# Mingtzge/PVE-MCC_for_unsignalized_intersection

Measured on AMD Instinct MI355X. Metric: env-steps/sec (vehicles x envs x steps/s) at 128 veh x 4096 envs, higher is better.
Workload: dtype f64

## Files before the change

### pve-mcc_for_unsignalized_intersection_amd/csrc/pve_tick_core.h

```cpp
#pragma once
#include "pve_types.h"
#include <math.h>
#include <string.h>
#include <type_traits>

#if defined(__HIP_DEVICE_COMPILE__)
#define PVE_AS4 __attribute__((address_space(4)))
#else
#define PVE_AS4
#endif
#if defined(__HIPCC__)
#undef PVE_HD
#define PVE_HD __device__ __forceinline__
#define PVE_DEVICE_CODE 1
#else
#define PVE_DEVICE_CODE 0
#endif

namespace pve {

typedef unsigned long long u64;

template <int NW> PVE_HD void vote(u64 *m, int t, bool f)
{
#if PVE_DEVICE_CODE
    u64 b = __ballot(f);
    if ((t & 63) == 0) m[t >> 6] = b;
#else
    if (f) m[t >> 6] |= 1ull << (t & 63);
#endif
}
template <int NW, int N> PVE_HD void vote_many(u64 *const (&m)[N], int t, const bool (&f)[N])
{
#if PVE_DEVICE_CODE
    u64 b[N];
#pragma unroll
    for (int k = 0; k < N; k++) b[k] = __ballot(f[k]);
    if ((t & 63) == 0) {
#pragma unroll
        for (int k = 0; k < N; k++) m[k][t >> 6] = b[k];
    }
#else
    for (int k = 0; k < N; k++) if (f[k]) m[k][t >> 6] |= 1ull << (t & 63);
#endif
}
PVE_HD bool mask_test(const u64 *m, int t) { return (m[t >> 6] >> (t & 63)) & 1ull; }
PVE_HD u64 below_sel(int rel)
{
    return rel >= 64 ? ~0ull : (rel > 0 ? ((1ull << (rel & 63)) - 1ull) : 0ull);
}
PVE_HD int popc_below(u64 w, int rel)
{
    const int r = rel < 0 ? 0 : (rel > 64 ? 64 : rel);
    const int c = __builtin_popcountll(w << ((64 - r) & 63));
    return r == 0 ? 0 : c;
}
template <int NW> PVE_HD int mask_below(const u64 *m, int t)
{
    int c = 0;
#pragma unroll
    for (int k = 0; k < NW; k++) c += popc_below(m[k], t - k * 64);
    return c;
}
template <int NW> PVE_HD int mask_rank(const u64 *m, int t)
{
#if PVE_DEVICE_CODE
    if constexpr (NW <= 2) {
    const u64 w0 = m[0], w1 = m[NW - 1];
    const bool up = NW > 1 && t >= 64;
    const u64 w = up ? w1 : w0;
    int c = (int)__builtin_amdgcn_mbcnt_hi((unsigned)(w >> 32), __builtin_amdgcn_mbcnt_lo((unsigned)w, 0u));
    c += up ? __builtin_popcountll(w0) : 0;
    return c;
    } else {
        static_assert(NW == 4, "mask_rank: 64, 128 or 256 slots");
        const int wi = t >> 6;
        u64 w = m[0];
        int c = 0;
#pragma unroll
        for (int k = 1; k < NW; k++) {
            const u64 mk = m[k];
            c += wi >= k ? __builtin_popcountll(m[k - 1]) : 0;
            w = wi == k ? mk : w;
        }
        return c + (int)__builtin_amdgcn_mbcnt_hi((unsigned)(w >> 32), __builtin_amdgcn_mbcnt_lo((unsigned)w, 0u));
    }
#else
    return mask_below<NW>(m, t);
#endif
}
template <int NW> PVE_HD int mask_count(const u64 *m)
{
    int c = 0;
#pragma unroll
    for (int k = 0; k < NW; k++) c += __builtin_popcountll(m[k]);
    return c;
}
template <int NW> PVE_HD int mask_prev(const u64 *m, int t)
{
    int best = -1;
#pragma unroll
    for (int k = 0; k < NW; k++) {
        const u64 b = m[k] & below_sel(t - k * 64);
        best = b ? (k * 64 + 63 - __builtin_clzll(b | 1ull)) : best;
    }
    return best;
}
PVE_HD void lds_add(int *p, int v)
{
#if PVE_DEVICE_CODE
    atomicAdd(p, v);
#else
    *p += v;
#endif
}
PVE_HD int lds_claim(int *p, int n)
{
#if PVE_DEVICE_CODE
    return atomicAdd(p, n);
#else
    int o = *p; *p += n; return o;
#endif
}
PVE_HD unsigned lds_xchg(unsigned *p, unsigned v)
{
#if PVE_DEVICE_CODE
    return __hip_atomic_exchange(p, v, __ATOMIC_ACQ_REL, __HIP_MEMORY_SCOPE_WORKGROUP);
#else
    const unsigned o = *p; *p = v; return o;
#endif
}
template <class T> PVE_HD void lds_store_relaxed(T *p, T v)
{
#if PVE_DEVICE_CODE
    __hip_atomic_store(p, v, __ATOMIC_RELAXED, __HIP_MEMORY_SCOPE_WORKGROUP);
#else
    *p = v;
#endif
}
template <bool COH, class T> PVE_HD T gld(const T *p)
{
#if PVE_DEVICE_CODE
    if constexpr (COH) {
        static_assert(sizeof(T) == 4 || sizeof(T) == 8, "gld: 4- or 8-byte scalars");
        if constexpr (sizeof(T) == 8) {
            const unsigned long long u = __hip_atomic_load((const unsigned long long *)p, __ATOMIC_RELAXED, __HIP_MEMORY_SCOPE_AGENT);
            T v; __builtin_memcpy(&v, &u, 8); return v;
        } else {
            const unsigned u = __hip_atomic_load((const unsigned *)p, __ATOMIC_RELAXED, __HIP_MEMORY_SCOPE_AGENT);
            T v; __builtin_memcpy(&v, &u, 4); return v;
        }
    } else return *p;
#else
    return *p;
#endif
}
template <class ROW> PVE_HD void gather_state(const ROW *const (&srcs)[NNB + 1], unsigned coh, ROW *dst)
{
#if PVE_DEVICE_CODE
    typedef float v4f __attribute__((ext_vector_type(4)));
    constexpr int CPR = (int)sizeof(ROW) * OBSW / 112;
    constexpr int NC = (NNB + 1) * CPR;
    v4f buf[7];
    auto fetch = [&](int c, v4f (&q)[7]) {
        const ROW *row = srcs[c / CPR];
        const char *sp = (const char *)row + 112 * (c % CPR);
        if (!row) {
#pragma unroll
            for (int i = 0; i < 7; i++) q[i] = v4f{0.f, 0.f, 0.f, 0.f};
        } else if ((coh >> (c / CPR)) & 1u) {
            asm volatile("global_load_dwordx4 %0, %7, off sc1\n\tglobal_load_dwordx4 %1, %7, off offset:16 sc1\n\t"
                         "global_load_dwordx4 %2, %7, off offset:32 sc1\n\tglobal_load_dwordx4 %3, %7, off offset:48 sc1\n\t"
                         "global_load_dwordx4 %4, %7, off offset:64 sc1\n\tglobal_load_dwordx4 %5, %7, off offset:80 sc1\n\t"
                         "global_load_dwordx4 %6, %7, off offset:96 sc1\n\ts_waitcnt vmcnt(0)"
                         : "=&v"(q[0]), "=&v"(q[1]), "=&v"(q[2]), "=&v"(q[3]), "=&v"(q[4]), "=&v"(q[5]), "=&v"(q[6]) : "v"(sp) : "memory");
        } else {
#pragma unroll
            for (int i = 0; i < 7; i++) q[i] = ((const v4f *)sp)[i];
        }
    };
#pragma unroll
    for (int c = 0; c < NC; c++) {
        fetch(c, buf);
        v4f *d4 = (v4f *)((char *)dst + 112 * c);
#pragma unroll
        for (int i = 0; i < 7; i++) d4[i] = buf[i];
    }
#else
    for (int q = 0; q <= NNB; q++)
        for (int k = 0; k < OBSW; k++) dst[q * OBSW + k] = srcs[q] ? srcs[q][k] : (ROW)0;
#endif
}
template <class W> PVE_HD int sidx_at(const W *s, int i)
{
    if constexpr (sizeof(W) == 4) return ((const uint16_t *)s)[2 * i];
    else return s[i];
}
PVE_HD void lds_or(int *p, int v)
{
#if PVE_DEVICE_CODE
    atomicOr(p, v);
#else
    *p |= v;
#endif
}
PVE_HD void lds_and(int *p, int v)
{
#if PVE_DEVICE_CODE
    atomicAnd(p, v);
#else
    *p &= v;
#endif
}
PVE_HD int wave_incl_scan(int t, int x, int *emu_acc)
{
#if PVE_DEVICE_CODE
    x += __builtin_amdgcn_mov_dpp(x, 0x111, 0xf, 0xf, true);
    x += __builtin_amdgcn_mov_dpp(x, 0x112, 0xf, 0xf, true);
    x += __builtin_amdgcn_mov_dpp(x, 0x114, 0xf, 0xf, true);
    x += __builtin_amdgcn_mov_dpp(x, 0x118, 0xf, 0xf, true);
    x += __builtin_amdgcn_update_dpp(0, x, 0x142, 0xa, 0xf, false);
    x += __builtin_amdgcn_update_dpp(0, x, 0x143, 0xc, 0xf, false);
    return x;
#else
    *emu_acc += x;
    return *emu_acc;
#endif
}
#if PVE_DEVICE_CODE
template <int CTRL, int ROW_MASK> PVE_HD double dpp_add_f64(double x)
{
    const int lo = __double2loint(x), hi = __double2hiint(x);
    int slo, shi;
    if (ROW_MASK == 0xf) {
        slo = __builtin_amdgcn_mov_dpp(lo, CTRL, 0xf, 0xf, true);
        shi = __builtin_amdgcn_mov_dpp(hi, CTRL, 0xf, 0xf, true);
    } else {
        slo = __builtin_amdgcn_update_dpp(0, lo, CTRL, ROW_MASK, 0xf, false);
        shi = __builtin_amdgcn_update_dpp(0, hi, CTRL, ROW_MASK, 0xf, false);
    }
    return x + __hiloint2double(shi, slo);
}
#endif
PVE_HD void block_sum(double *red, int t, double x)
{
#if PVE_DEVICE_CODE
    x = dpp_add_f64<0x111, 0xf>(x);
    x = dpp_add_f64<0x112, 0xf>(x);
    x = dpp_add_f64<0x114, 0xf>(x);
    x = dpp_add_f64<0x118, 0xf>(x);
    x = dpp_add_f64<0x142, 0xa>(x);
    x = dpp_add_f64<0x143, 0xc>(x);
    if ((t & 63) == 63) red[t >> 6] = x;
#else
    red[0] += x;
#endif
}

PVE_HD void block_sum_sparse(double *red, int t, bool has, double x)
{
#if PVE_DEVICE_CODE
    if (__builtin_amdgcn_ballot_w64(has) == 0) {
        if ((t & 63) == 63) red[t >> 6] = 0.0;
        return;
    }
#endif
    block_sum(red, t, has ? x : 0.0);
}

#ifdef PVE_SELECT_CLAMPS
PVE_HD double dmax(double a, double b) { return (a > b) ? a : b; }
PVE_HD double dmin(double a, double b) { return (a < b) ? a : b; }
#else
PVE_HD double dmax(double a, double b) { return __builtin_fmax(a, b); }
PVE_HD double dmin(double a, double b) { return __builtin_fmin(a, b); }
#endif

#ifdef PVE_WIDE_INDEX
template <int PER, class T> PVE_HD T *env_at(T *base, int env, int idx) { return base + ((size_t)env * PER + (size_t)idx); }
#else
template <int PER, class T> PVE_HD T *env_at(T *base, int env, int idx)
{
    return (T *)((char *)(base + (size_t)env * PER) + (unsigned)(idx * (int)sizeof(T)));
}
#endif

PVE_HD int mul24(int a, int b)
{
#if PVE_DEVICE_CODE && !defined(PVE_NO_RANGE_ASSUME)
    return __mul24(a, b);
#else
    return a * b;
#endif
}
PVE_HD int mad24(int a, int b, int c)
{
#if PVE_DEVICE_CODE && !defined(PVE_NO_RANGE_ASSUME)
    return __mul24(a, b) + c;
#else
    return a * b + c;
#endif
}

template <int CAP> using slot_t = typename std::conditional<(CAP <= 128), uint8_t, uint16_t>::type;
template <int CAP> constexpr int SLOT_NONE = CAP <= 128 ? 255 : 0xFFFF;
template <int CAP> struct Homes {
    static_assert(CAP <= 128, "HOME: id_info[1] is packed into one byte of h_sv (no HOME build at 256 slots)");
    double h_jerk_sum[CAP], h_closer[CAP];
    int h_id[CAP], h_sv[CAP], h_count[CAP];
};
template <int CAP> struct HomesOff {};
struct HomeRegs { double jerk_sum, closer, vir_dis; int id, sv, count; };
template <int CAP, bool LJ = (CAP == 128), bool HOME_ = false, int POOL_ = (HOME_ ? 304 * CAP / 128 : 5 * CAP)>
struct Shared : std::conditional<HOME_, Homes<CAP>, HomesOff<CAP>>::type {
    static constexpr int NW = CAP / 64;
    static constexpr bool HOME = HOME_;
    static_assert(!HOME_ || (POOL_ * 4 >= 2 * CAP * 4 + CAP + 1 && POOL_ >= CAP && POOL_ % 8 == 0), "HOME: the staging overlays need 2 CAP ints + CAP + 1 bytes of s_idx");
    static constexpr bool PIN_READS = true;
    static constexpr int POOL = POOL_;
    static constexpr bool DIRECT = (CAP == 64);
    static constexpr bool DENSE = true;
    EnvHeader hd;
    double p[CAP], v[CAP + 1], a[CAP + 1];
    union {
        struct { double p1[CAP], v1[CAP]; };
        double u_vd[POOL];
    };
    double virdis[CAP];
    int cnt[CAP];
    alignas(8) unsigned s_idx[DIRECT ? 1 : POOL];
    double s_vd[DIRECT ? POOL : 1];
    alignas(8) uint8_t u_slot[POOL];
    enum { SF_JERK = 0, SF_JERK_SUM, SF_VIR_DIS, SF_CLOSER_P, SF_P, SF_V, SF_A };
    template <int K> PVE_HD double *stf()
    {
        if (HOME) return K == SF_JERK ? u_vd + CAP : (K == SF_P ? p : (K == SF_V ? v : a));
        return K < 4 ? u_vd + (K + 1) * CAP : (K == SF_P ? u_vd : (K == SF_V ? v : a));
    }
    PVE_HD slot_t<CAP> *keep_pre() { return (slot_t<CAP> *)(DIRECT ? (uint8_t *)s_vd + 7 * CAP * 4 : (uint8_t *)s_idx + 2 * CAP * 4); }
    PVE_HD uint8_t *fxcode() { return u_list + CAP; }
    PVE_HD slot_t<CAP> *chain() { return (slot_t<CAP> *)u_slot; }
    template <int K> PVE_HD int *sti()
    {
        if (DIRECT) return (int *)s_vd + K * CAP;
        if (HOME) return K == I_STEP ? (int *)s_idx : (K == I_META ? (int *)s_idx + CAP : cnt);
        return K < 2 ? (int *)s_idx + K * CAP : (K < 4 ? (int *)p + (K - 2) * CAP : (K == 4 ? cnt : (K == 5 ? (int *)u_slot : (int *)(u_list + CAP))));
    }
    int acc_passed_steps, acc_collisions;
    union {
        int16_t pref[NL * 5];
        int16_t hdr[CAP];
    };
    union {
        uint8_t bb[CAP];
        uint8_t rew_ovr[CAP];
    };
    u64 m_alive[NW], m_ctl[NW];
    union {
        int nfin[NL];
        struct {
            u64 m_del[NW], m_fin[NW], m_ctlnow[NW], m_coll[NW];
            union { u64 m_lead[NW]; u64 m_keep[NW]; };
            u64 m_spawn[NW];
        };
    };
    uint8_t s_slot[DIRECT ? POOL : 1];
    union {
        alignas(8) uint8_t u_list[POOL];
        uint8_t lk_slot[POOL];
    };
    union {
        uint8_t mypos[CAP];
        uint8_t cyc_off[CAP];
    };
    uint8_t slot_of[CAP];
    int16_t cstart[NL + 1];
#if !PVE_DEVICE_CODE
    int emu_scan;
#endif
    int16_t loff[NL + 1];
    union {
        alignas(8) int16_t segoff[NL][5];
        struct { double red_reward[NW], red_jerk[NW]; };
    };
    uint8_t lane_of[CAP + 1];
    static constexpr bool HAS_LJ = LJ;
    int lj[HAS_LJ ? CAP + 1 : 1];
    union {
        float xy32[CAP][2];
        double act_next[CAP];
    };
    double tabA[2][4], tabB[2][4], tabC[2][4];
    alignas(4) uint8_t l2lp[NL][4];
    int lead_n;
    static_assert(POOL < (1 << 16), "s_idx: entry | tag << 16");
    static_assert((CAP + 1) * sizeof(slot_t<CAP>) <= POOL, "chain() in u_slot");
    static_assert(HOME_ || 5 * CAP <= POOL, "stf<>(): the EARLY staging doubles in u_vd[0 .. 5 CAP)");
    static_assert(DIRECT || HOME_ || (CAP * 4 <= POOL && CAP + CAP * 4 <= POOL), "sti<5>() in u_slot, sti<6>() in u_list[CAP ..)");
    static_assert(DIRECT ? 7 * CAP * 4 + (CAP + 1) * sizeof(slot_t<CAP>) <= POOL * sizeof(double)
                         : 2 * CAP * 4 + (CAP + 1) * sizeof(slot_t<CAP>) <= POOL * 4, "keep_pre() behind the EARLY staging ints");
};

struct Regs {
    double p, v, a, jerk, jerk_sum, vir_dis, closer_p;
    double a0, a1;
    double reward;
    double kv[NNB];
    int kr[NNB];
    int id, seq, vnum, step, count, meta;
    int lane, j;
    int hdr;
    int hit, coll_seen, coll_fin;
    int alive, ctl, del, fin;
    int cyc;
    int intent, route, ord;
    int mmask;
    int dctl, ds, dlane;
    double dp, djerk, dcloser;
    double act;
    double next_arr;
    double act_nx;
};
struct FinCarry {
    int still, meta;
    int new_slot;
    int ls;
    int sp_slot, sp_id, sp_vnum;
    int sp_int;
    int n_post, n_sp;
    int n_ctl;
};
struct CRegs {
    double p, v, a, jerk, jerk_sum, vir_dis, closer_p;
    int id, seq, vnum, step, count, meta, hdr_word, alive;
    double obsrow[OBSW];
};

PVE_HD void sincos_q1(double x, double &sn, double &cs)
{
    const double hp = 1.5707963267948966;
    const bool fold = x > 0.7853981633974483;
    const double y = fold ? (hp - x) : x;
    const double z = y * y;
    double ps = -7.6471637318198164759e-13;
    ps = ps * z + 1.6059043836821614599e-10;
    ps = ps * z - 2.5052108385441718775e-08;
    ps = ps * z + 2.7557319223985890653e-06;
    ps = ps * z - 1.9841269841269841270e-04;
    ps = ps * z + 8.3333333333333333333e-03;
    ps = ps * z - 1.6666666666666666667e-01;
    const double s1 = y + y * z * ps;
    double pc = 4.7794773323873852974e-14;
    pc = pc * z - 1.1470745597729724714e-11;
    pc = pc * z + 2.0876756987868098979e-09;
    pc = pc * z - 2.7557319223985890653e-07;
    pc = pc * z + 2.4801587301587301587e-05;
    pc = pc * z - 1.3888888888888888889e-03;
    pc = pc * z + 4.1666666666666666667e-02;
    const double c1 = 1.0 - 0.5 * z + z * z * pc;
    sn = fold ? c1 : s1;
    cs = fold ? s1 : c1;
}

#if PVE_DEVICE_CODE
#define PVE_PIN(x) asm volatile("" : "+v"(x))
#else
#define PVE_PIN(x) ((void)0)
#endif

PVE_HD double sel2(double a0, double a1, bool second)
{
#if PVE_DEVICE_CODE
    asm volatile("" : "+s"(a0), "+s"(a1));
#endif
    return second ? a1 : a0;
}
PVE_HD double sel3(const PVE_AS4 double (&a)[3], int i)
{
    double a0 = a[0], a1 = a[1], a2 = a[2];
#if PVE_DEVICE_CODE
    asm volatile("" : "+s"(a0), "+s"(a1), "+s"(a2));
#endif
    return i == 0 ? a0 : (i == 1 ? a1 : a2);
}
PVE_HD double sel4(const PVE_AS4 double (&a)[4], int i)
{
    double a0 = a[0], a1 = a[1], a2 = a[2], a3 = a[3];
#if PVE_DEVICE_CODE
    asm volatile("" : "+s"(a0), "+s"(a1), "+s"(a2), "+s"(a3));
#endif
    return i == 0 ? a0 : (i == 1 ? a1 : (i == 2 ? a2 : a3));
}

PVE_HD void get_xy(const PVE_AS4 Const &c, double p, int lane, double &X, double &Y)
{
    const double cw = c.cw;
    const int m = lane % 3;
    const double Lb = sel2(c.inbox[0], c.inbox[2], m == 2);
    const bool before = p > Lb, inside = !before && p > 0;
    const bool arc = (m != 1) && inside;
    double sn, cs;
    sincos_q1(arc ? ((Lb - p) / Lb * c.arc_k / 2) : 0.0, sn, cs);
    const double p0y = (m == 0) ? cw : 5 * cw, pry = (m == 0) ? -6 * cw : 6 * cw;
    const double p0x = 6 * cw, prx = 6 * cw;
    const double ax = (m == 0) ? (prx + (p0x - prx) * cs - (p0y - pry) * sn) : (prx + (p0x - prx) * cs + (p0y - pry) * sn);
    const double ay = (m == 0) ? (pry + (p0y - pry) * cs + (p0x - prx) * sn) : (pry + (p0y - pry) * cs - (p0x - prx) * sn);
    const double bx = p - Lb + 6 * cw, by = p0y;
    const double ex = (m == 0) ? -cw : 5 * cw;
    const double ey = (m == 0) ? (-6 * cw + p) : (6 * cw - p);
    double x = before ? bx : (inside ? ax : ex);
    double y = before ? by : (inside ? ay : ey);
    if (m == 1) { x = p - 6 * cw; y = 3 * cw; }
    const double rc = sel4(c.rot_cos, lane / 3), rs = sel4(c.rot_sin, lane / 3);
    X = x * rc - y * rs;
    Y = y * rc + x * rs;
}

PVE_HD float frcp(float x)
{
#if PVE_DEVICE_CODE
    return __builtin_amdgcn_rcpf(x);
#else
    return 1.0f / x;
#endif
}
PVE_HD void get_xy_f32(const PVE_AS4 Const &c, double pd, int lane, float &X, float &Y)
{
    const float cw = (float)c.cw, p = (float)pd;
    const int m = lane % 3;
    const float Lb = (float)sel2(c.inbox[0], c.inbox[2], m == 2);
    const bool before = p > Lb, inside = !before && p > 0.f;
    float ra = (m != 1 && inside) ? ((Lb - p) * (1.5707965f * frcp(Lb))) : 0.f;
    const bool fold = ra > 0.78539816f;
    const float y0 = fold ? (1.5707964f - ra) : ra, z = y0 * y0;
    const float s1 = y0 + y0 * z * (-1.6666667e-1f + z * (8.3333338e-3f + z * (-1.9841270e-4f + z * 2.7557319e-6f)));
    const float c1 = 1.f + z * (-0.5f + z * (4.1666668e-2f + z * (-1.3888889e-3f + z * 2.4801587e-5f)));
    const float sn = fold ? c1 : s1, cs = fold ? s1 : c1;
    const float p0y = (m == 0) ? cw : 5.f * cw, pry = (m == 0) ? -6.f * cw : 6.f * cw, prx = 6.f * cw;
    const float ax = (m == 0) ? (prx - (p0y - pry) * sn) : (prx + (p0y - pry) * sn);
    const float ay = pry + (p0y - pry) * cs;
    float x = before ? (p - Lb + 6.f * cw) : (inside ? ax : ((m == 0) ? -cw : 5.f * cw));
    float y = before ? p0y : (inside ? ay : ((m == 0) ? (-6.f * cw + p) : (6.f * cw - p)));
    if (m == 1) { x = p - 6.f * cw; y = 3.f * cw; }
    const int q = lane / 3;
    const bool odd = (q & 1) != 0;
    const float xr = odd ? -y : x, yr = odd ? x : y;
    X = (q & 2) ? -xr : xr;
    Y = (q & 2) ? -yr : yr;
}

PVE_HD double exp_m2_0(double x)
{
    const double k = rint(x * 1.4426950408889634074);
    double r = __builtin_fma(-k, 6.93147180369123816490e-01, x);
    r = __builtin_fma(-k, 1.90821492927058770002e-10, r);
    double p = 1.0 / 479001600.0;
    p = __builtin_fma(p, r, 1.0 / 39916800.0);
    p = __builtin_fma(p, r, 1.0 / 3628800.0);
    p = __builtin_fma(p, r, 1.0 / 362880.0);
    p = __builtin_fma(p, r, 1.0 / 40320.0);
    p = __builtin_fma(p, r, 1.0 / 5040.0);
    p = __builtin_fma(p, r, 1.0 / 720.0);
    p = __builtin_fma(p, r, 1.0 / 120.0);
    p = __builtin_fma(p, r, 1.0 / 24.0);
    p = __builtin_fma(p, r, 1.0 / 6.0);
    p = __builtin_fma(p, r, 0.5);
    p = __builtin_fma(p, r, 1.0);
    p = __builtin_fma(p, r, 1.0);
    return ldexp(p, (int)k);
}
PVE_HD double value_div(double x, double y)
{
#if PVE_DEVICE_CODE
    double r = __builtin_amdgcn_rcp(y);
    r = __builtin_fma(__builtin_fma(-y, r, 1.0), r, r);
    r = __builtin_fma(__builtin_fma(-y, r, 1.0), r, r);
    return x * r;
#else
    return x / y;
#endif
}
PVE_HD double reward_coth_term(double t_distance)
{
    const double u = exp_m2_0(-0.5 * t_distance);
    const double den = u - 1.0;
    return den == 0.0 ? -INFINITY : value_div(u + 1.0, den);
}
PVE_HD double reward_log_term(double z)
{
    int e;
    double m = frexp(z, &e);
    const bool lo = m < 0.70710678118654752;
    m = lo ? m + m : m;
    e = lo ? e - 1 : e;
    const double f = m - 1.0;
    const double s = value_div(f, 2.0 + f);
    const double w = s * s;
    double q = 1.0 / 19.0;
    q = __builtin_fma(q, w, 1.0 / 17.0);
    q = __builtin_fma(q, w, 1.0 / 15.0);
    q = __builtin_fma(q, w, 1.0 / 13.0);
    q = __builtin_fma(q, w, 1.0 / 11.0);
    q = __builtin_fma(q, w, 1.0 / 9.0);
    q = __builtin_fma(q, w, 1.0 / 7.0);
    q = __builtin_fma(q, w, 1.0 / 5.0);
    q = __builtin_fma(q, w, 1.0 / 3.0);
    q = __builtin_fma(q, w, 1.0);
    return __builtin_fma((double)e, 0.69314718055994530942, (s + s) * q);
}

PVE_HD bool key_less(double d1, double v1, int r1, double d2, double v2, int r2)
{
    return d1 < d2 || (d1 == d2 && (v1 < v2 || (v1 == v2 && r1 < r2)));
}

PVE_HD double div_const(double x, double b, double rb)
{
    const double q = x * rb;
    const double r = __builtin_fma(-q, b, x);
    return __builtin_fma(r, rb, q);
}
PVE_HD int brake_needed(const PVE_AS4 Const &c, double p, double v, double fp, double fv)
{
    const double d_safe = v * 0.4 + div_const(v * v - fv * fv, c.two_abs_am, c.inv_two_abs_am) -
                          div_const((v - fv) * c.vm, c.abs_am, c.inv_abs_am);
    return ((fv < v) & (p - fp < d_safe)) ? 1 : 0;
}

PVE_HD int slot_lane(const EnvHeader &hd, int t)
{
    int lane = 0;
#pragma unroll
    for (int L = 1; L < NL; L++) lane += (t >= hd.lane_start[L]) ? 1 : 0;
    return lane;
}

template <int CAP, class ShT = Shared<CAP>> struct Tick {
    typedef ShT Sh;
    static constexpr int NW = CAP / 64;

    template <bool COH = false, bool COHA = false>
    static PVE_HD void ph_load(const PVE_AS4 Const &c, const PVE_AS4 Params &P, int env, int t, Sh &sh, Regs &r,
                               const double *act0 = nullptr, bool use_act0 = false)
    {
        const EnvHeader &gh = P.headers[env];
        {
            const int *src = (const int *)&gh;
            int *dst = (int *)&sh.hd;
            for (int w = t + 2; w < (int)(sizeof(EnvHeader) / 4); w += CAP) dst[w] = gld<COH>(src + w);
        }
        if (t == 0) sh.hd.current_time = gld<COH>(&gh.current_time) + c.deltaT;
        const int N = gld<COH>(&gh.n_alive);
        const size_t g = (size_t)env * CAP + t;
        r.alive = t < N;
        r.jerk = 0;
        r.p = r.v = r.a = r.jerk_sum = r.vir_dis = r.closer_p = 0;
        r.id = r.seq = r.vnum = r.step = r.count = r.meta = 0;
        r.act = 0;
        const double *acts = use_act0 ? act0 : P.actions;
        if (t < 64 || t < N) {
            if (acts) r.act = gld<COHA>(acts + g);
            r.p = gld<COH>(P.f64[F_P] + g); r.v = gld<COH>(P.f64[F_V] + g); r.a = gld<COH>(P.f64[F_A] + g);
            r.meta = gld<COH>(P.i32[I_META] + g); r.step = gld<COH>(P.i32[I_STEP] + g);
            r.jerk_sum = gld<COH>(P.f64[F_JERK_SUM] + g); r.vir_dis = gld<COH>(P.f64[F_VIR_DIS] + g);
            r.closer_p = gld<COH>(P.f64[F_CLOSER_P] + g);
            r.id = gld<COH>(P.i32[I_ID] + g); r.seq = gld<COH>(P.i32[I_SEQ] + g); r.vnum = gld<COH>(P.i32[I_VNUM] + g);
            r.count = gld<COH>(P.i32[I_COUNT] + g);
        }
        sh.cnt[t] = 0;
        if (t == 0) {
            sh.acc_passed_steps = 0; sh.acc_collisions = 0; sh.lead_n = 0;
            sh.v[CAP] = 0; sh.a[CAP] = 0; sh.lane_of[CAP] = 0;
            if constexpr (Sh::HAS_LJ) sh.lj[CAP] = 0;
        }
        if (t < 8) {
            sh.tabA[t >> 2][t & 3] = c.vdA[t >> 2][t & 3];
            sh.tabB[t >> 2][t & 3] = c.vdB[t >> 2][t & 3];
            sh.tabC[t >> 2][t & 3] = c.vdC[t >> 2][t & 3];
        }
        if (t < NL * 4) {
            const int L = c.l2l[t >> 2][t & 3];
            sh.l2lp[t >> 2][t & 3] = (uint8_t)((L < 0 ? 15 : L) | ((c.l2l_inv[t >> 2][t & 3] & 3) << 4) | ((L < 0 ? 0 : (L % 3) & 1) << 6));
        }
    }

    static PVE_HD void ph_home_store(int t, Sh &sh, Regs &r)
    {
        if constexpr (Sh::HOME) {
            sh.h_jerk_sum[t] = r.jerk_sum; sh.h_closer[t] = r.closer_p;
            sh.h_id[t] = r.id; sh.h_sv[t] = (r.seq << 8) | (r.vnum & 0xFF); sh.h_count[t] = r.count;
            sh.p[t] = r.p; sh.v[t] = r.v; sh.a[t] = r.a; sh.virdis[t] = r.vir_dis; sh.act_next[t] = r.act;
        }
    }

    static PVE_HD void outcome(const PVE_AS4 Const &c, double p, double v, double a, bool ctl, double &pn, double &vn)
    {
        pn = p - v * c.deltaT - 0.5 * a * c.dt2;
        const double x = v + a * c.deltaT;
        vn = dmin(dmax(c.vm, x), c.vM);
        if (!ctl) vn = c.v0;
    }
    static PVE_HD double clip_a(const PVE_AS4 Const &c, double x)
    {
        return dmin(c.aM, dmax(x, c.am));
    }
    static PVE_HD void ph_step1(const PVE_AS4 Const &c, const PVE_AS4 Params &P, int env, int t, Sh &sh, Regs &r)
    {
        r.ctl = 0; r.lane = 0; r.j = 0; r.a0 = r.a1 = 0;
        if constexpr (Sh::HOME) {
            r.p = sh.p[t]; r.v = sh.v[t]; r.a = sh.a[t]; r.act = sh.act_next[t];
        }
        if (r.alive) {
            const int lane = (r.meta >> M_LANE_SHIFT) & M_LANE_MASK;
            r.lane = lane; r.j = t - sh.hd.lane_start[lane];
            sh.lane_of[t] = (uint8_t)lane;
            if constexpr (Sh::HAS_LJ) sh.lj[t] = (lane << 16) | r.j;
            r.ctl = (r.meta & M_CONTROL) ? 1 : 0;
            double act = r.act;
            if (P.mask_uncontrolled && !r.ctl) act = 0.0;
            double target = clip_a(c, act);
            if ((r.meta & M_LOCK) && (r.meta & (M_LOCKA_POS | M_LOCKA_NEG)) && r.p > 70)
                target = r.a + ((r.meta & M_LOCKA_POS) ? 1.0 : -1.0);
            r.meta &= ~(M_LOCK | M_LOCKA_POS | M_LOCKA_NEG);
            bool ovr = ((sh.hd.head_valid >> lane) & 1) && sh.hd.head_lane[lane] == lane &&
                       sh.hd.head_j[lane] == r.j;
            ovr = ovr || (lane % 3 == 2);
            r.a0 = clip_a(c, ovr ? c.aM : target);
            r.a1 = clip_a(c, ovr ? c.aM : c.am);
            double pn, vn;
            outcome(c, r.p, r.v, r.a0, r.ctl, pn, vn); sh.p[t] = pn; sh.v[t] = vn;
            outcome(c, r.p, r.v, r.a1, r.ctl, pn, vn); sh.p1[t] = pn; sh.v1[t] = vn;
        }
        {
            u64 *const ms[2] = {sh.m_alive, sh.m_ctl};
            const bool fs[2] = {r.alive != 0, r.alive && r.ctl};
            vote_many<NW>(ms, t, fs);
        }
    }

    static PVE_HD void ph_step2(const PVE_AS4 Const &c, int t, Sh &sh, Regs &r)
    {
        int bb = 0;
        if (r.alive && r.j > 0 && r.ctl && mask_test(sh.m_ctl, t - 1)) {
            bb = brake_needed(c, r.p, r.v, sh.p[t - 1], sh.v[t - 1]) |
                 (brake_needed(c, r.p, r.v, sh.p1[t - 1], sh.v1[t - 1]) << 1);
        }
        sh.bb[t] = (uint8_t)bb;
        if constexpr (Sh::DENSE) {
            if (r.alive && r.ctl) sh.slot_of[mask_rank<NW>(sh.m_ctl, t)] = (uint8_t)t;
        }
    }

    static PVE_HD void ph_step3(const PVE_AS4 Const &c, int t, Sh &sh, Regs &r, bool last = false)
    {
        if (r.alive) {
            int k = t;
            while (sh.bb[k] == 1 || sh.bb[k] == 2) k--;
            int br = sh.bb[k] & 1;
            for (int q = k + 1; q <= t; q++) br = (sh.bb[q] >> br) & 1;
            double an = br ? r.a1 : r.a0;
            r.jerk = an - r.a;
            r.a = an;
            r.p = br ? sh.p1[t] : sh.p[t];
            r.v = br ? sh.v1[t] : sh.v[t];
            r.step += 1;
            if constexpr (Sh::HOME) {
                if (r.ctl) { sh.virdis[t] = r.jerk; sh.h_jerk_sum[t] = sh.h_jerk_sum[t] + fabs(r.jerk * c.inv_dt); }
                else if (last) sh.act_next[t] = r.jerk;
            }
        }
    }
    static PVE_HD void ph_step3_publish(int t, Sh &sh, Regs &r)
    {
        if (r.alive) { sh.p[t] = r.p; sh.v[t] = r.v; sh.a[t] = r.a; }
    }

    static PVE_HD void ph_lists_a(const PVE_AS4 Const &c, int t, Sh &sh)
    {
        int cnt = 0;
        if (t < NL * 5) {
            const int d = t / 5, k = t - d * 5;
            const int Lp = (k == 0) ? d : (int)(sh.l2lp[d][k == 0 ? 0 : k - 1] & 15);
            if (Lp != 15) {
                const int b0 = mask_below<NW>(sh.m_ctl, sh.hd.lane_start[Lp]);
                cnt = mask_below<NW>(sh.m_ctl, sh.hd.lane_start[Lp + 1]) - b0;
                if (k == 0) { sh.cstart[d] = (int16_t)b0; if (d == NL - 1) sh.cstart[NL] = (int16_t)(b0 + cnt); }
            }
        }
#if PVE_DEVICE_CODE
        const int incl = wave_incl_scan(t, cnt, nullptr);
#else
        const int incl = wave_incl_scan(t, cnt, &sh.emu_scan);
#endif
        if (t < NL * 5) sh.pref[t] = (int16_t)incl;
    }
    static PVE_HD void ph_lists_b(int t, Sh &sh)
    {
        if (t < NL * 5) {
            const int d = t / 5, k = t - d * 5;
            const int base = d ? sh.pref[5 * d - 1] : 0;
            const int mine = t ? sh.pref[t - 1] : 0;
            sh.segoff[d][k] = (int16_t)(mine - base);
            if (k == 0) { sh.loff[d] = (int16_t)base; sh.nfin[d] = sh.pref[t] - base; }
        }
        if (t == NL * 5) sh.loff[NL] = sh.pref[NL * 5 - 1];
    }

    static PVE_HD int group_end(const Sh &sh, int d0)
    {
        if constexpr (!Sh::HOME) return NL;
        else {
            const int b = sh.loff[d0];
            if (sh.loff[NL] - b <= Sh::POOL) return NL;
            int d1 = d0 + 1;
            while (d1 < NL && sh.loff[d1 + 1] - b <= Sh::POOL) d1++;
            return d1;
        }
    }
    static PVE_HD void ph_build(const PVE_AS4 Const &c, int t, Sh &sh, Regs &r)
    {
        ph_build_prep(c, t, sh, r);
        ph_build_fill<false>(c, t, sh, r, 0, NL);
    }
    static PVE_HD void ph_build_prep(const PVE_AS4 Const &c, int t, Sh &sh, Regs &r)
    {
        sh.rew_ovr[t] = 0; sh.hdr[t] = -1;
        if constexpr (!Sh::HOME) sh.virdis[t] = (r.alive && r.ctl) ? r.jerk : r.vir_dis;
        r.dctl = t < mask_count<NW>(sh.m_ctl);
        r.ds = 0; r.dlane = 0; r.dp = 0;
        if (!r.dctl) return;
        const int sl = sh.slot_of[t];
        const int lane = sh.lane_of[sl];
        const double p = sh.p[sl];
        r.ds = sl; r.dlane = lane; r.dp = p;
        get_xy_f32(c, p, lane, sh.xy32[sl][0], sh.xy32[sl][1]);
    }
    template <bool GRP = Sh::HOME>
    static PVE_HD void ph_build_fill(const PVE_AS4 Const &c, int t, Sh &sh, Regs &r, int d0, int d1)
    {
        if (!r.dctl) return;
        const int sl = r.ds, lane = r.dlane;
        const double p = r.dp;
        const int gb = GRP ? (int)sh.loff[d0] : 0;
        const int q = t - sh.cstart[lane];
        if (!GRP || (lane >= d0 && lane < d1)) {
            const int e = sh.loff[lane] + q - gb;
            sh.u_vd[e] = p; sh.u_slot[e] = (uint8_t)sl; sh.u_list[e] = (uint8_t)lane;
        }
        if (lane % 3 == 2) return;
        const int pk = *(const int *)sh.l2lp[lane];
        int d[4], kk[4], mk[4];
#pragma unroll
        for (int k = 0; k < 4; k++) {
            d[k] = (pk >> (8 * k)) & 15; kk[k] = (pk >> (8 * k + 4)) & 3; mk[k] = (pk >> (8 * k + 4)) & 7;
        }
        double tA[4], tB[4], tC[4]; int lo[4], so[4];
#pragma unroll
        for (int k = 0; k < 4; k++) {
            tA[k] = (&sh.tabA[0][0])[mk[k]]; tB[k] = (&sh.tabB[0][0])[mk[k]]; tC[k] = (&sh.tabC[0][0])[mk[k]];
            lo[k] = sh.loff[d[k]]; so[k] = sh.segoff[d[k]][kk[k] + 1];
        }
#pragma unroll
        for (int k = 0; k < 4; k++) { PVE_PIN(tA[k]); PVE_PIN(tB[k]); PVE_PIN(tC[k]); PVE_PIN(lo[k]); PVE_PIN(so[k]); }
#pragma unroll
        for (int k = 0; k < 4; k++) {
            const double delta = p - tA[k] + tB[k];
            const double vd = (delta > 0) ? (tC[k] + delta) : INFINITY;
            const int e = lo[k] + so[k] + q - gb;
            if constexpr (GRP) { if (d[k] < d0 || d[k] >= d1) continue; }
            sh.u_vd[e] = vd; sh.u_slot[e] = (uint8_t)sl; sh.u_list[e] = (uint8_t)d[k];
            lds_add(&sh.nfin[d[k]], (delta > 0) ? 1 : 0);
        }
    }

    template <bool GRP = false>
    static PVE_HD void ph_rank(int t, Sh &sh, int salt = 0, int d0 = 0, int d1 = NL)
    {
        const int gb = GRP ? (int)sh.loff[d0] : 0;
        const int M = (GRP ? (int)sh.loff[d1] : (int)sh.loff[NL]) - gb;
        const unsigned tag = Sh::DIRECT ? 0u : (((unsigned)sh.hd.ticks + (unsigned)salt * 0x9E37u) << 16);
        for (int e = t; e < M; e += CAP) {
            const int d = sh.u_list[e];
            const double vd = sh.u_vd[e];
            if (!(vd < INFINITY)) continue;
            const int lo = sh.loff[d] - gb, hi = sh.loff[d + 1] - gb;
            int pos = 0, eq = 0;
            int f = lo;
            for (; f + 8 <= hi; f += 8) {
                const double w0 = sh.u_vd[f], w1 = sh.u_vd[f + 1], w2 = sh.u_vd[f + 2], w3 = sh.u_vd[f + 3];
                const double w4 = sh.u_vd[f + 4], w5 = sh.u_vd[f + 5], w6 = sh.u_vd[f + 6], w7 = sh.u_vd[f + 7];
                pos += (w0 < vd) + (w1 < vd) + (w2 < vd) + (w3 < vd) + (w4 < vd) + (w5 < vd) + (w6 < vd) + (w7 < vd);
                if (Sh::DIRECT) eq += (w0 == vd) + (w1 == vd) + (w2 == vd) + (w3 == vd) + (w4 == vd) + (w5 == vd) + (w6 == vd) + (w7 == vd);
            }
            if (f < hi) {
                const int n = hi - f;
                double w[7];
                const double *uv = sh.u_vd;
#pragma unroll
                for (int k = 0; k < 7; k++) w[k] = uv[f + k];
#pragma unroll
                for (int k = 0; k < 7; k++) { pos += (k < n) & (w[k] < vd); if (Sh::DIRECT) eq += (k < n) & (w[k] == vd); }
            }
            const int myslot = sh.u_slot[e];
            const int nown = sh.cstart[d + 1] - sh.cstart[d];
            if (Sh::DIRECT) {
                if (eq > 1)
                    for (f = lo; f < hi; f++) pos += (sh.u_vd[f] == vd && sh.u_slot[f] < myslot) ? 1 : 0;
                sh.s_vd[lo + pos] = vd; sh.s_slot[lo + pos] = (uint8_t)myslot;
                if (e - lo < nown) sh.mypos[myslot] = (uint8_t)pos;
            } else {
                if (e - lo < nown) lds_store_relaxed(&sh.mypos[myslot], (uint8_t)pos);
                const unsigned old = lds_xchg(&sh.s_idx[Sh::DIRECT ? 0 : lo + pos], tag | (unsigned)e);
                if ((old & 0xFFFF0000u) == tag) {
                    for (f = lo; f < hi; f++) {
                        if (!(sh.u_vd[f] == vd)) continue;
                        const int sf = sh.u_slot[f];
                        int rk = 0;
                        for (int g = lo; g < hi; g++) rk += (sh.u_vd[g] == vd && sh.u_slot[g] < sf) ? 1 : 0;
                        lds_store_relaxed(&sh.s_idx[Sh::DIRECT ? 0 : lo + pos + rk], tag | (unsigned)f);
                        if (f - lo < nown) lds_store_relaxed(&sh.mypos[sf], (uint8_t)(pos + rk));
                    }
                }
            }
        }
    }

    static PVE_HD unsigned f32_bits(float x)
    {
#if PVE_DEVICE_CODE
        return __float_as_uint(x);
#else
        unsigned u; memcpy(&u, &x, 4); return u;
#endif
    }
    static PVE_HD unsigned umin(unsigned a, unsigned b) { return a < b ? a : b; }
    static PVE_HD unsigned umax(unsigned a, unsigned b) { return a < b ? b : a; }
    static PVE_HD void walk_window(Sh &sh, int base, int n, int s, double ps, Regs &r, int &pr, double &pvd)
    {
        const auto *sidx = sh.s_idx + base;
#define sv(pos_) (Sh::DIRECT ? sh.s_vd[Sh::DIRECT ? base + (pos_) : 0] : sh.u_vd[sidx_at(sidx, pos_)])
#define ss(pos_) (Sh::DIRECT ? sh.s_slot[Sh::DIRECT ? base + (pos_) : 0] : sh.u_slot[sidx_at(sidx, pos_)])
        const int last = n - 1;
        double lraw[NNB + 1], rraw[NNB];
        int prs = -1;
#pragma unroll
        for (int i = 0; i < NNB + 1; i++) {
            const int pos = s - 1 - i, pc = pos >= 0 ? pos : 0;
            lraw[i] = sv(pc);
            if (i == 0) prs = (int)ss(pc);
        }
#pragma unroll
        for (int i = 0; i < NNB; i++) {
            const int pos = s + 1 + i, pc = pos <= last ? pos : last;
            rraw[i] = sv(pc);
        }
        if (Sh::PIN_READS) {
#pragma unroll
            for (int i = 0; i < NNB + 1; i++) PVE_PIN(lraw[i]);
#pragma unroll
            for (int i = 0; i < NNB; i++) PVE_PIN(rraw[i]);
            PVE_PIN(prs);
        }
        pr = (s > 0) ? prs : -1; pvd = (s > 0) ? lraw[0] : 0.0;
        double dl[NNB + 1];
#pragma unroll
        for (int i = 0; i < NNB + 1; i++) dl[i] = fabs(lraw[i] - ps);
        bool amb = false;
#pragma unroll
        for (int i = 1; i < NNB + 1; i++) amb = amb | ((s - 1 - i >= 0) & (dl[i] == dl[i - 1]));
        unsigned kl[NNB], kq[NNB];
#pragma unroll
        for (int i = 0; i < NNB; i++) {
            const unsigned cl = (unsigned)i, cr = 8u + (unsigned)i;
            const unsigned bl = f32_bits((float)dl[i]), br = f32_bits((float)fabs(rraw[i] - ps));
            kl[i] = (s - 1 - i >= 0) ? ((bl & ~15u) | cl) : (0xFF800000u | (cl << 4) | cl);
            kq[i] = (s + 1 + i <= last) ? ((br & ~15u) | cr) : (0xFF800000u | (cr << 4) | cr);
        }
        unsigned w[NNB], acc = ~0u;
#pragma unroll
        for (int i = 0; i < NNB; i++) {
            const unsigned a = kl[i], b = kq[NNB - 1 - i];
            w[i] = umin(a, b);
            acc = umin(acc, a ^ b);
        }
#define PVE_CE(A, B) { const unsigned lo_ = umin(w[A], w[B]), hi_ = umax(w[A], w[B]); w[A] = lo_; w[B] = hi_; }
        PVE_CE(0, 5) PVE_CE(1, 3) PVE_CE(2, 4)
        PVE_CE(1, 2) PVE_CE(3, 4)
        PVE_CE(0, 3) PVE_CE(2, 5)
        PVE_CE(0, 1) PVE_CE(2, 3) PVE_CE(4, 5)
        PVE_CE(1, 2) PVE_CE(3, 4)
#undef PVE_CE
        amb = amb | (acc < 16u);
        int ei[NNB], sl[NNB]; double vv[NNB];
#pragma unroll
        for (int k = 0; k < NNB; k++) {
            const int code = (int)(w[k] & 15u);
            const int pos = (code & 8) ? (s - 7 + code) : (s - 1 - code);
            const int pc = ((int)w[k] >= 0) ? pos : 0;
            ei[k] = Sh::DIRECT ? (base + pc) : sidx_at(sidx, pc);
        }
#pragma unroll
        for (int k = 0; k < NNB; k++) PVE_PIN(ei[k]);
#pragma unroll
        for (int k = 0; k < NNB; k++) {
            sl[k] = Sh::DIRECT ? (int)sh.s_slot[Sh::DIRECT ? ei[k] : 0] : (int)sh.u_slot[ei[k]];
            vv[k] = Sh::DIRECT ? sh.s_vd[Sh::DIRECT ? ei[k] : 0] : sh.u_vd[ei[k]];
        }
#pragma unroll
        for (int k = 0; k < NNB; k++) { PVE_PIN(sl[k]); PVE_PIN(vv[k]); }
        double dk[NNB];
#pragma unroll
        for (int k = 0; k < NNB; k++) dk[k] = fabs(vv[k] - ps);
        bool dec = false;
#pragma unroll
        for (int k = 1; k < NNB; k++) dec = dec | (((int)w[k] >= 0) & (dk[k] < dk[k - 1]));
#if PVE_DEVICE_CODE
        if (__builtin_amdgcn_ballot_w64(dec) != 0)
#else
        if (dec)
#endif
        {
#pragma unroll
            for (int k = 1; k < NNB; k++) {
                const bool sw = ((int)w[k] >= 0) & (dk[k] < dk[k - 1]);
                const double td = sw ? dk[k - 1] : dk[k], tv = sw ? vv[k - 1] : vv[k]; const int ts = sw ? sl[k - 1] : sl[k];
                dk[k - 1] = sw ? dk[k] : dk[k - 1]; vv[k - 1] = sw ? vv[k] : vv[k - 1]; sl[k - 1] = sw ? sl[k] : sl[k - 1];
                dk[k] = td; vv[k] = tv; sl[k] = ts;
            }
#pragma unroll
            for (int k = 1; k < NNB; k++) amb = amb | (((int)w[k] >= 0) & (dk[k] < dk[k - 1]));
        }
        if (!amb) {
#pragma unroll
            for (int k = 0; k < NNB; k++) {
                const bool ok = (int)w[k] >= 0;
                r.kr[k] = ok ? sl[k] : -1;
                r.kv[k] = ok ? vv[k] : 0.0;
            }
        } else {
            walk_window_exact(sh, base, n, s, ps, r);
        }
#undef sv
#undef ss
    }

    static PVE_HD void walk_window_exact(Sh &sh, int base, int n, int s, double ps, Regs &r)
    {
        const auto *sidx = sh.s_idx + base;
#define sv(pos_) (Sh::DIRECT ? sh.s_vd[Sh::DIRECT ? base + (pos_) : 0] : sh.u_vd[sidx_at(sidx, pos_)])
#define ss(pos_) (Sh::DIRECT ? sh.s_slot[Sh::DIRECT ? base + (pos_) : 0] : sh.u_slot[sidx_at(sidx, pos_)])
        const int last = n - 1;
        double lv[NNB + 1], rv[NNB];
#pragma unroll
        for (int i = 0; i < NNB + 1; i++) { const int pos = s - 1 - i; lv[i] = pos >= 0 ? sv(pos >= 0 ? pos : 0) : -INFINITY; }
#pragma unroll
        for (int i = 0; i < NNB; i++) { const int pos = s + 1 + i; rv[i] = pos <= last ? sv(pos <= last ? pos : last) : INFINITY; }
        const double pvd = lv[0];
        bool tie = false;
#pragma unroll
        for (int i = 1; i < NNB + 1; i++) tie = tie || (s - 1 - i >= 0 && fabs(lv[i] - ps) == fabs(lv[i - 1] - ps));
        double cd[NNB]; int cc[NNB];
#pragma unroll
        for (int i = 0; i < NNB; i++) {
            const double dl = (s - 1 - i >= 0) ? fabs(lv[i] - ps) : INFINITY;
            const int j = NNB - 1 - i;
            const double dr = (s + 1 + j <= last) ? fabs(rv[j] - ps) : INFINITY;
            const bool takeL = dl <= dr;
            cd[i] = takeL ? dl : dr; cc[i] = takeL ? i : (8 + j);
        }
#define PVE_CE(A, B)                                                                            \
        {                                                                                       \
            const bool sw = cd[B] < cd[A];                                                      \
            const double td = sw ? cd[A] : cd[B]; const int tc = sw ? cc[A] : cc[B];            \
            cd[A] = sw ? cd[B] : cd[A]; cc[A] = sw ? cc[B] : cc[A];                             \
            cd[B] = td; cc[B] = tc;                                                             \
        }
        PVE_CE(0, 5) PVE_CE(1, 3) PVE_CE(2, 4)
        PVE_CE(1, 2) PVE_CE(3, 4)
        PVE_CE(0, 3) PVE_CE(2, 5)
        PVE_CE(0, 1) PVE_CE(2, 3) PVE_CE(4, 5)
        PVE_CE(1, 2) PVE_CE(3, 4)
#undef PVE_CE
#pragma unroll
        for (int k = 1; k < NNB; k++) tie = tie || (cd[k] == cd[k - 1] && cd[k] < INFINITY);
        if (!tie) {
#pragma unroll
            for (int k = 0; k < NNB; k++) {
                const bool ok = cd[k] < INFINITY;
                const int code = cc[k];
                const int pos = (code < 8) ? (s - 1 - code) : (s + 1 + (code - 8));
                r.kr[k] = ok ? (int)ss(ok ? pos : 0) : -1;
                r.kv[k] = ok ? sv(ok ? pos : 0) : 0.0;
            }
        } else {
#pragma unroll
            for (int k = 0; k < NNB; k++) { r.kr[k] = -1; r.kv[k] = 0; }
            int hi = s - 1, lo = hi, cur, rr = s + 1;
            if (hi >= 0) { const double dh = fabs(pvd - ps); while (lo > 0 && fabs(sv(lo - 1) - ps) == dh) lo--; }
            cur = lo;
            for (int k = 0; k < NNB; k++) {
                const bool hasL = hi >= 0;
                const bool hasR = rr < n;
                if (!(hasL || hasR)) break;
                double vR = INFINITY;
                if (hasR) vR = sv(rr);
                double vL = 0;
                if (hasL) vL = sv(cur);
                const double dL = fabs(vL - ps), dR = fabs(vR - ps);
                const bool takeL = hasL && (!hasR || dL <= dR);
                int slot; double vv;
                if (takeL) {
                    slot = ss(cur); vv = vL;
                    cur++;
                    if (cur > hi) {
                        hi = lo - 1; lo = hi;
                        if (hi >= 0) { const double dh = fabs(sv(hi) - ps); while (lo > 0 && fabs(sv(lo - 1) - ps) == dh) lo--; }
                        cur = lo;
                    }
                } else {
                    slot = ss(rr); vv = vR;
                    rr++;
                }
#pragma unroll
                for (int q = 0; q < NNB; q++) if (q == k) { r.kr[q] = slot; r.kv[q] = vv; }
            }
        }
#undef sv
#undef ss
    }

    static PVE_HD void ph_scan_init(Regs &r)
    {
        r.reward = 0; r.hit = 0; r.hdr = -1; r.djerk = 0;
#pragma unroll
        for (int k = 0; k < NNB; k++) { r.kr[k] = -1; r.kv[k] = 0; }
    }
    static PVE_HD void ph_scan(const PVE_AS4 Const &c, int t, Sh &sh, Regs &r)
    {
        ph_scan_init(r);
        ph_scan_lists<false>(c, t, sh, r, 0, NL);
    }
    template <bool GRP = Sh::HOME>
    static PVE_HD void ph_scan_lists(const PVE_AS4 Const &c, int t, Sh &sh, Regs &r, int d0, int d1)
    {
        const int gb = GRP ? (int)sh.loff[d0] : 0;
        const bool rebuilt = t < NL && sh.hd.lane_start[t < NL ? t + 1 : 0] > sh.hd.lane_start[t < NL ? t : 0] &&
                             (!GRP || (t >= d0 && t < d1));
        bool hvalid = false;
        if (rebuilt) {
            const int base = sh.loff[t] - gb;
            if (sh.nfin[t] > 0) {
                const int hr = Sh::DIRECT ? sh.s_slot[Sh::DIRECT ? base : 0] : sh.u_slot[sidx_at(sh.s_idx, base)];
                hvalid = true;
                int hl = sh.lane_of[hr];
                sh.hd.head_lane[t] = hl;
                sh.hd.head_j[t] = hr - sh.hd.lane_start[hl];
            }
        }
#if PVE_DEVICE_CODE
        {
            const unsigned mr = (unsigned)__ballot(rebuilt), mv = (unsigned)__ballot(hvalid);
            if (t == 0) sh.hd.head_valid = (sh.hd.head_valid & ~(int)mr) | (int)mv;
        }
#else
        if (rebuilt) { if (hvalid) sh.hd.head_valid |= 1 << t; else sh.hd.head_valid &= ~(1 << t); }
#endif
        if (!r.dctl) return;
        const int sl = r.ds, lane = r.dlane;
        if constexpr (GRP) { if (lane < d0 || lane >= d1) return; }
        const double ps = r.dp;
        const int base = sh.loff[lane] - gb, n = sh.nfin[lane];
        int pr; double pvd;
        walk_window(sh, base, n, sh.mypos[sl], ps, r, pr, pvd);
        r.hdr = pr;
        const double vd = (pr >= 0) ? (ps - pvd) : 100.0;
        r.djerk = sh.virdis[sl];
        sh.hdr[sl] = (int16_t)pr;
        sh.virdis[sl] = vd;
    }

    static PVE_HD void ph_reward(const PVE_AS4 Const &c, int t, Sh &sh, Regs &r)
    {
        r.dcloser = 150;
        if (!r.dctl) return;
        const int sl = r.ds, lane = r.dlane;
        const double ps = r.dp;
        const double myv = sh.v[sl];
        double t_distance = 2, d_distance = 10;
        const int n0 = r.kr[0];
        if (n0 >= 0) {
            const double vdn = r.kv[0];
            d_distance = fabs(ps - vdn);
            r.dcloser = vdn;
            if (d_distance != 0) t_distance = (ps - vdn) / (myv - sh.v[n0] + 0.0001);
        }
        double r_ = 0;
        if (0 < t_distance && t_distance < 4) r_ += reward_coth_term(t_distance);
        const double jd = r.djerk * c.inv_dt;
        r_ -= jd * jd * (3.0 / 3600.0);
        if (d_distance < 10) {
            double q1 = d_distance * 0.1, q2 = q1 * q1;
            r_ += reward_log_term(q2 * q2 * q1 + 0.00001);
        }
        r_ += (myv - c.vm) * c.inv_span * 2.0;
        r.reward = dmin(dmax(r_, -20.0), 20.0);
        bool near = false;
        if (n0 >= 0) {
            const float fx = sh.xy32[n0][0] - sh.xy32[sl][0], fy = sh.xy32[n0][1] - sh.xy32[sl][1];
            const float lim = (float)c.collision_thr + 0.05f;
            near = fx * fx + fy * fy < lim * lim;
        }
        if (near) {
            double ax, ay, bx, by;
            get_xy(c, ps, lane, ax, ay);
            get_xy(c, sh.p[n0], sh.lane_of[n0], bx, by);
            double dx = bx - ax, dy = by - ay;
            double dxy = sqrt(dx * dx + dy * dy);
            if (fabs(dxy) < c.collision_thr) {
                lds_add(&sh.cnt[sl], 1);
                lds_add(&sh.cnt[n0], (sl < n0) ? 1 : (1 << 16));
            }
        }
// ... 807 lines not shown
```

Before: 23.04 billion.

## Rank list entries in pairs so each thread compares two keys per scan

In the non-direct shared layout, the rank phase now assigns each thread a pair of adjacent entries within a lane list instead of one entry. The thread scans the list once and counts positions for both keys, halving the LDS reads per comparison. To support this, pair offsets per lane are computed with an extra wave scan in ph_lists_b and packed with the entry offsets into a new lpo array, and u_list is indexed by pair cell. This adds scan and bookkeeping work and may lower parallelism when lists are short.

```diff
diff --git a/pve-mcc_for_unsignalized_intersection_amd/csrc/pve_tick_core.h b/pve-mcc_for_unsignalized_intersection_amd/csrc/pve_tick_core.h
--- a/pve-mcc_for_unsignalized_intersection_amd/csrc/pve_tick_core.h
+++ b/pve-mcc_for_unsignalized_intersection_amd/csrc/pve_tick_core.h
@@ -20,6 +20,10 @@
 namespace pve {
 
 typedef unsigned long long u64;
+
+#if !PVE_DEVICE_CODE && defined(PVE_EMU_DIAG)
+inline int emu_diag_list_len[64], emu_diag_ties[2];
+#endif
 
 template <int NW> PVE_HD void vote(u64 *m, int t, bool f)
 {
@@ -358,12 +362,15 @@
     u64 m_alive[NW], m_ctl[NW];
     union {
         int nfin[NL];
+        int nfin_lpo[DIRECT ? NL : 2 * NL + 1];
         struct {
             u64 m_del[NW], m_fin[NW], m_ctlnow[NW], m_coll[NW];
             union { u64 m_lead[NW]; u64 m_keep[NW]; };
             u64 m_spawn[NW];
         };
     };
+    PVE_HD int *lpo() { return nfin_lpo + (DIRECT ? 0 : NL); }
+    PVE_HD const int *lpo() const { return nfin_lpo + (DIRECT ? 0 : NL); }
     uint8_t s_slot[DIRECT ? POOL : 1];
     union {
         alignas(8) uint8_t u_list[POOL];
@@ -796,14 +803,30 @@
     }
     static PVE_HD void ph_lists_b(int t, Sh &sh)
     {
+        int d = 0, k = 0, end = 0, np = 0;
         if (t < NL * 5) {
-            const int d = t / 5, k = t - d * 5;
+            d = t / 5; k = t - d * 5;
             const int base = d ? sh.pref[5 * d - 1] : 0;
             const int mine = t ? sh.pref[t - 1] : 0;
+            end = sh.pref[t];
             sh.segoff[d][k] = (int16_t)(mine - base);
-            if (k == 0) { sh.loff[d] = (int16_t)base; sh.nfin[d] = sh.pref[t] - base; }
+            if (k == 0) { sh.loff[d] = (int16_t)base; sh.nfin[d] = end - base; }
+            if (k == 4) np = (end - base + 1) >> 1;
         }
         if (t == NL * 5) sh.loff[NL] = sh.pref[NL * 5 - 1];
+#if !PVE_DEVICE_CODE && defined(PVE_EMU_DIAG)
+        if (t == NL * 5 && CAP == 128) for (int q = 0; q < NL; q++) { const int n = sh.loff[q + 1] - sh.loff[q]; emu_diag_list_len[n < 63 ? n : 63]++; }
+#endif
+        if constexpr (!Sh::DIRECT) {
+#if PVE_DEVICE_CODE
+            const int pin = wave_incl_scan(t, np, nullptr);
+#else
+            if (t == 0) sh.emu_scan = 0;
+            const int pin = wave_incl_scan(t, np, &sh.emu_scan);
+#endif
+            if (t < NL * 5 && k == 4) sh.lpo()[d + 1] = end | (pin << 16);
+            if (t == 0) sh.lpo()[0] = 0;
+        }
     }
 
     static PVE_HD int group_end(const Sh &sh, int d0)
@@ -817,6 +840,10 @@
             return d1;
         }
     }
+    static PVE_HD int lp_word(const Sh &sh, int d) { if constexpr (Sh::DIRECT) return sh.loff[d]; else return sh.lpo()[d]; }
+    static PVE_HD int lp_lo(int w) { return Sh::DIRECT ? w : (w & 0xFFFF); }
+    static PVE_HD int lp_pair(int w) { return Sh::DIRECT ? 0 : (int)((unsigned)w >> 16); }
+    static PVE_HD int lp_cell(int w, int in, int e, int pgb) { return Sh::DIRECT ? e : lp_pair(w) - pgb + (in >> 1); }
     static PVE_HD void ph_build(const PVE_AS4 Const &c, int t, Sh &sh, Regs &r)
     {
         ph_build_prep(c, t, sh, r);
@@ -841,11 +868,13 @@
         if (!r.dctl) return;
         const int sl = r.ds, lane = r.dlane;
         const double p = r.dp;
-        const int gb = GRP ? (int)sh.loff[d0] : 0;
+        const int gw = GRP ? lp_word(sh, d0) : 0;
+        const int gb = lp_lo(gw), pgb = lp_pair(gw);
         const int q = t - sh.cstart[lane];
         if (!GRP || (lane >= d0 && lane < d1)) {
-            const int e = sh.loff[lane] + q - gb;
-            sh.u_vd[e] = p; sh.u_slot[e] = (uint8_t)sl; sh.u_list[e] = (uint8_t)lane;
+            const int lw = lp_word(sh, lane);
+            const int e = lp_lo(lw) + q - gb;
+            sh.u_vd[e] = p; sh.u_slot[e] = (uint8_t)sl; sh.u_list[lp_cell(lw, q, e, pgb)] = (uint8_t)lane;
         }
         if (lane % 3 == 2) return;
         const int pk = *(const int *)sh.l2lp[lane];
@@ -858,7 +887,7 @@
 #pragma unroll
         for (int k = 0; k < 4; k++) {
             tA[k] = (&sh.tabA[0][0])[mk[k]]; tB[k] = (&sh.tabB[0][0])[mk[k]]; tC[k] = (&sh.tabC[0][0])[mk[k]];
-            lo[k] = sh.loff[d[k]]; so[k] = sh.segoff[d[k]][kk[k] + 1];
+            lo[k] = lp_word(sh, d[k]); so[k] = sh.segoff[d[k]][kk[k] + 1];
         }
 #pragma unroll
         for (int k = 0; k < 4; k++) { PVE_PIN(tA[k]); PVE_PIN(tB[k]); PVE_PIN(tC[k]); PVE_PIN(lo[k]); PVE_PIN(so[k]); }
@@ -866,9 +895,9 @@
         for (int k = 0; k < 4; k++) {
             const double delta = p - tA[k] + tB[k];
             const double vd = (delta > 0) ? (tC[k] + delta) : INFINITY;
-            const int e = lo[k] + so[k] + q - gb;
+            const int e = lp_lo(lo[k]) + so[k] + q - gb;
             if constexpr (GRP) { if (d[k] < d0 || d[k] >= d1) continue; }
-            sh.u_vd[e] = vd; sh.u_slot[e] = (uint8_t)sl; sh.u_list[e] = (uint8_t)d[k];
+            sh.u_vd[e] = vd; sh.u_slot[e] = (uint8_t)sl; sh.u_list[lp_cell(lo[k], so[k] + q, e, pgb)] = (uint8_t)d[k];
             lds_add(&sh.nfin[d[k]], (delta > 0) ? 1 : 0);
         }
     }
@@ -876,21 +905,24 @@
     template <bool GRP = false>
     static PVE_HD void ph_rank(int t, Sh &sh, int salt = 0, int d0 = 0, int d1 = NL)
     {
-        const int gb = GRP ? (int)sh.loff[d0] : 0;
-        const int M = (GRP ? (int)sh.loff[d1] : (int)sh.loff[NL]) - gb;
-        const unsigned tag = Sh::DIRECT ? 0u : (((unsigned)sh.hd.ticks + (unsigned)salt * 0x9E37u) << 16);
+        if constexpr (Sh::DIRECT) ph_rank_entries(t, sh);
+        else ph_rank_pairs<GRP>(t, sh, salt, d0, d1);
+    }
+    static PVE_HD void ph_rank_entries(int t, Sh &sh)
+    {
+        const int M = sh.loff[NL];
         for (int e = t; e < M; e += CAP) {
             const int d = sh.u_list[e];
             const double vd = sh.u_vd[e];
             if (!(vd < INFINITY)) continue;
-            const int lo = sh.loff[d] - gb, hi = sh.loff[d + 1] - gb;
+            const int lo = sh.loff[d], hi = sh.loff[d + 1];
             int pos = 0, eq = 0;
             int f = lo;
             for (; f + 8 <= hi; f += 8) {
                 const double w0 = sh.u_vd[f], w1 = sh.u_vd[f + 1], w2 = sh.u_vd[f + 2], w3 = sh.u_vd[f + 3];
                 const double w4 = sh.u_vd[f + 4], w5 = sh.u_vd[f + 5], w6 = sh.u_vd[f + 6], w7 = sh.u_vd[f + 7];
                 pos += (w0 < vd) + (w1 < vd) + (w2 < vd) + (w3 < vd) + (w4 < vd) + (w5 < vd) + (w6 < vd) + (w7 < vd);
-                if (Sh::DIRECT) eq += (w0 == vd) + (w1 == vd) + (w2 == vd) + (w3 == vd) + (w4 == vd) + (w5 == vd) + (w6 == vd) + (w7 == vd);
+                eq += (w0 == vd) + (w1 == vd) + (w2 == vd) + (w3 == vd) + (w4 == vd) + (w5 == vd) + (w6 == vd) + (w7 == vd);
             }
             if (f < hi) {
                 const int n = hi - f;
@@ -899,25 +931,68 @@
 #pragma unroll
                 for (int k = 0; k < 7; k++) w[k] = uv[f + k];
 #pragma unroll
-                for (int k = 0; k < 7; k++) { pos += (k < n) & (w[k] < vd); if (Sh::DIRECT) eq += (k < n) & (w[k] == vd); }
+                for (int k = 0; k < 7; k++) { pos += (k < n) & (w[k] < vd); eq += (k < n) & (w[k] == vd); }
             }
             const int myslot = sh.u_slot[e];
             const int nown = sh.cstart[d + 1] - sh.cstart[d];
-            if (Sh::DIRECT) {
-                if (eq > 1)
-                    for (f = lo; f < hi; f++) pos += (sh.u_vd[f] == vd && sh.u_slot[f] < myslot) ? 1 : 0;
-                sh.s_vd[lo + pos] = vd; sh.s_slot[lo + pos] = (uint8_t)myslot;
-                if (e - lo < nown) sh.mypos[myslot] = (uint8_t)pos;
-            } else {
+            if (eq > 1)
+                for (f = lo; f < hi; f++) pos += (sh.u_vd[f] == vd && sh.u_slot[f] < myslot) ? 1 : 0;
+            sh.s_vd[Sh::DIRECT ? lo + pos : 0] = vd; sh.s_slot[Sh::DIRECT ? lo + pos : 0] = (uint8_t)myslot;
+            if (e - lo < nown) sh.mypos[myslot] = (uint8_t)pos;
+        }
+    }
+    template <bool GRP>
+    static PVE_HD void ph_rank_pairs(int t, Sh &sh, int salt, int d0, int d1)
+    {
+        const int gw = GRP ? sh.lpo()[d0] : 0;
+        const int gb = lp_lo(gw), pgb = lp_pair(gw);
+        const int NP = lp_pair(GRP ? sh.lpo()[d1] : sh.lpo()[NL]) - pgb;
+        const unsigned tag = ((unsigned)sh.hd.ticks + (unsigned)salt * 0x9E37u) << 16;
+        const double *uv = sh.u_vd;
+        for (int i = t; i < NP; i += CAP) {
+            const int d = sh.u_list[i];
+            const int lw = sh.lpo()[d];
+            const int lo = lp_lo(lw) - gb, hi = lp_lo(sh.lpo()[d + 1]) - gb;
+            const int e0 = lo + 2 * (i - (lp_pair(lw) - pgb));
+            const double vd0 = uv[e0];
+            double vd1 = uv[e0 + 1];
+            if (e0 + 1 >= hi) vd1 = INFINITY;
+            if (!(vd0 < INFINITY) && !(vd1 < INFINITY)) continue;
+            int pos0 = 0, pos1 = 0;
+            int f = lo;
+            for (; f + 8 <= hi; f += 8) {
+                const double w0 = uv[f], w1 = uv[f + 1], w2 = uv[f + 2], w3 = uv[f + 3];
+                const double w4 = uv[f + 4], w5 = uv[f + 5], w6 = uv[f + 6], w7 = uv[f + 7];
+                pos0 += (w0 < vd0) + (w1 < vd0) + (w2 < vd0) + (w3 < vd0) + (w4 < vd0) + (w5 < vd0) + (w6 < vd0) + (w7 < vd0);
+                pos1 += (w0 < vd1) + (w1 < vd1) + (w2 < vd1) + (w3 < vd1) + (w4 < vd1) + (w5 < vd1) + (w6 < vd1) + (w7 < vd1);
+            }
+            if (f < hi) {
+                const int n = hi - f;
+                double w[7];
+#pragma unroll
+                for (int k = 0; k < 7; k++) w[k] = uv[f + k];
+#pragma unroll
+                for (int k = 0; k < 7; k++) { pos0 += (k < n) & (w[k] < vd0); pos1 += (k < n) & (w[k] < vd1); }
+            }
+            const int nown = sh.cstart[d + 1] - sh.cstart[d];
+#pragma unroll
+            for (int h = 0; h < 2; h++) {
+                const int e = e0 + h, pos = h ? pos1 : pos0;
+                const double vd = h ? vd1 : vd0;
+                if (!(vd < INFINITY)) continue;
+                const int myslot = sh.u_slot[e];
                 if (e - lo < nown) lds_store_relaxed(&sh.mypos[myslot], (uint8_t)pos);
-                const unsigned old = lds_xchg(&sh.s_idx[Sh::DIRECT ? 0 : lo + pos], tag | (unsigned)e);
+                const unsigned old = lds_xchg(&sh.s_idx[lo + pos], tag | (unsigned)e);
                 if ((old & 0xFFFF0000u) == tag) {
+#if !PVE_DEVICE_CODE && defined(PVE_EMU_DIAG)
+                    emu_diag_ties[(h == 1 && vd0 == vd1) ? 0 : 1]++;
+#endif
                     for (f = lo; f < hi; f++) {
-                        if (!(sh.u_vd[f] == vd)) continue;
+                        if (!(uv[f] == vd)) continue;
                         const int sf = sh.u_slot[f];
                         int rk = 0;
-                        for (int g = lo; g < hi; g++) rk += (sh.u_vd[g] == vd && sh.u_slot[g] < sf) ? 1 : 0;
-                        lds_store_relaxed(&sh.s_idx[Sh::DIRECT ? 0 : lo + pos + rk], tag | (unsigned)f);
+                        for (int g = lo; g < hi; g++) rk += (uv[g] == vd && sh.u_slot[g] < sf) ? 1 : 0;
+                        lds_store_relaxed(&sh.s_idx[lo + pos + rk], tag | (unsigned)f);
                         if (f - lo < nown) lds_store_relaxed(&sh.mypos[sf], (uint8_t)(pos + rk));
                     }
                 }
```

After: 23.46 billion, median of 6. +1.8%, better.
